# lucabaldesi/srsRAN

Measured on AMD Instinct MI355X. Metric: PDSCH decoded Mbps + code-blocks/sec, 20 MHz TM4 QAM256, 1/2/4/8 GPU, higher is better.
Workload: dtype fp32+int16; 1 GPU; srslte_ue_dl chain from time-domain I/Q: 2048 subframes/GPU/batch, 20 MHz (100 PRB), TM4 2x2 spatial multiplexing, 2 codewords QAM256 TBS 97896 (C=16, K=6144), MMSE+CSI, max 10 half-its with CRC early stop, 40 dB crossed 2x2 channel, every subframe distinct (GPU eNodeB generator, keyed by global subframe index); 3 PHY worker threads (own ue_dl / stream / softbuffers each) decode alternate batches,; subframes_per_gpu_batch=2048, code_blocks_per_gpu_batch=65536, workers_per_gpu=3, parallelism=dp1

## Files before the change

srsran_amd/csrc/tdec_kernels.hip:

```cpp
#include <hip/hip_runtime.h>

#include <atomic>
#include <stdint.h>
#include <stdlib.h>

#include "crc_device.h"
#include "tdec_internal.h"
#include "tdec_trellis.h"

namespace mi355 {

__device__ __forceinline__ uint32_t hi_lo(uint32_t a, uint32_t b) { return __builtin_amdgcn_alignbit(b, a, 16); }
__device__ __forceinline__ uint32_t from_prev(uint32_t v)
{
  return (uint32_t)__builtin_amdgcn_update_dpp(0, (int)v, 0x111, 0xf, 0xf, true);
}
__device__ __forceinline__ uint32_t from_next(uint32_t v)
{
  return (uint32_t)__builtin_amdgcn_update_dpp(0, (int)v, 0x101, 0xf, 0xf, true);
}

__device__ __forceinline__ void bm_set(uint32_t* bm, uint32_t m, bool v)
{
  __hip_atomic_fetch_or(&bm[m >> 5], (uint32_t)v << ((m & 31u) ^ 7u), __ATOMIC_RELAXED, __HIP_MEMORY_SCOPE_WORKGROUP);
}

template <int NL>
__device__ __forceinline__ void tdec_fused_check(const TdecWinArgs& a, int cb, int l, int K, const uint32_t* bm,
                                                 const uint32_t (*t4)[4][256])
{
  const DlschCheckArgs& c      = a.chk;
  const CbDesc&         d      = c.desc[cb];
  const uint32_t        nbytes = (uint32_t)K / 8, chunk = nbytes / NL;
  const int             pi     = d.C > 1 ? 1 : 0;
  const uint8_t*        bytes  = (const uint8_t*)bm;
  uint32_t              crc    = crc24_words(bytes + l * chunk, chunk, t4[pi]);
  crc = gf2_mulmod24(crc, c.scale[128 + 8 * pi + l], pi ? c.crc24b->poly : c.crc24a->poly);
#pragma unroll
  for (int o = NL / 2; o >= 1; o >>= 1) crc ^= (uint32_t)__shfl_xor((int)crc, o, 64);
  const bool ok  = crc == 0;
  const bool fin = ok || c.h + 1 == c.max_its;
  if (fin) {
    uint8_t*       dst  = c.data + d.data_off + (size_t)d.cb * d.rlen / 8;
    const uint32_t nb   = d.nb;
    const uint32_t head = min(nb, (4u - (uint32_t)((uintptr_t)dst & 3u)) & 3u);
    const uint32_t nw   = (nb - head) / 4, tail0 = head + 4 * nw;
    for (uint32_t i = l; i < head; i += NL) dst[i] = bytes[i];
    for (uint32_t i = tail0 + l; i < nb; i += NL) dst[i] = bytes[i];
    uint32_t* dw = (uint32_t*)(dst + head);
    const uint32_t sh = head;
    for (uint32_t w = l; w < nw; w += NL) {
      const uint32_t lo = bm[w + sh / 4], hi = bm[w + sh / 4 + 1];
      dw[w]             = sh ? __builtin_amdgcn_alignbyte(hi, lo, sh) : lo;
    }
    if (l == 0) {
      c.its[cb] = c.h + 1;
      if (ok) {
        c.done[cb]       = 1;
        c.sb_crc[d.slot] = 1;
      } else {
        c.done[cb] = 2;
      }
    }
  }
  const uint64_t un = __builtin_amdgcn_ballot_w64(l == 0 && !fin);
  if (un && (threadIdx.x & 63) == (uint32_t)__builtin_ctzll(un)) flag_set(c.next);
}


#define WG_AT(arr, j) (arr)[((size_t)grp * Lp + (j)) * 64 + q]

#define TDEC_BM_WORDS (8 * 193)
__shared__ uint32_t tdec_tx_lds[4][2][TDEC_SEG * 64];
__shared__ uint32_t tdec_ym_lds[4][8 * SB_ROWMASK_WORDS];
__shared__ uint32_t tdec_bm_lds[4 * TDEC_BM_WORDS];
__shared__ int16_t  tdec_stg_lds[4][TDEC_SEG * 128];
__shared__ uint32_t tdec_stg_row[4][TDEC_SEG];

#ifndef TDEC_WAVES_PER_EU
#define TDEC_WAVES_PER_EU 2
#endif
template <int NSB, int SEG, int MODE, int DIAG, bool FULL, int OUTK, bool GI = false, bool TX = false>
__device__ __forceinline__ void tdec_win_body(const TdecWinArgs& a, const int gl,
                                              const uint32_t (*crc_t4)[4][256] = nullptr)
{
  constexpr int NL = NSB / 2;
  constexpr int G  = 64 / NL;
  static_assert(!TX || (NSB == 16 && FULL && SEG == 8), "TX loads need 8-lane rows and whole 8-step segments");
  static_assert((DIAG >= 0 && DIAG <= 4) || DIAG == 20, "DIAG values the body knows");
  const int     grp = __builtin_amdgcn_readfirstlane(gl >> 6), q = gl & 63;
  const int     cbg = q / NL, l = q % NL;
  if constexpr (!TX) {
    if (grp * G + cbg >= a.ncb) return;
    if (a.done && a.done[grp * G + cbg]) return;
  }
  if (a.remaining && *a.remaining == 0) return;

  const int  L = a.L, Lp = a.Lp, nseg = a.nseg;
  constexpr bool CL     = DIAG == 20;
  constexpr bool dec2   = MODE == 2;
  constexpr bool has_ap = MODE == 1;

  const int       cb   = grp * G + cbg;
  const int       K    = L * NSB;
  const size_t    bidx = a.in_idx ? a.in_idx[cb] : (size_t)cb;
  const uint32_t* in32 = (const uint32_t*)(a.in + bidx * a.in_stride);
  const size_t    wg0  = (size_t)grp * Lp * 64 + q;
  const uint32_t* X    = dec2 ? a.E + wg0 : (GI ? a.gS + wg0 : in32 + l);
  const int       xs   = (dec2 || GI) ? 64 : NL;
  const uint32_t* Y    = GI ? a.gP + wg0 : in32 + (dec2 ? (K + 32) : (K + 32) / 2) + l;
  const int       ys   = GI ? 64 : NL;
  const uint32_t* AP   = a.A1 + wg0;
  uint32_t*       ck   = a.ckpt + (size_t)grp * nseg * 8 * 64 + q;

  const uint4*    txin  = nullptr;
  if constexpr (TX) {
    const int txc = grp * G + ((q >> 1) & 7);
    txin = (const uint4*)(a.in + (a.in_idx ? (size_t)a.in_idx[txc] : (size_t)txc) * a.in_stride) + (2 * (q >> 4) + (q & 1));
  }
  const int       txoX  = 0;
  const int       txoY  = (dec2 ? (L * NSB + 32) : (L * NSB + 32) / 2) / 4;
  uint32_t*       txb   = nullptr;
  if constexpr (TX) {
    txb = &tdec_tx_lds[threadIdx.x >> 6][0][0];
  }
  constexpr bool RMK = NSB == 16 && !GI;
  uint32_t*      ymask = nullptr;
  if constexpr (RMK) {
    ymask = tdec_ym_lds[threadIdx.x >> 6];
#pragma unroll
    for (int w = l; w < SB_ROWMASK_WORDS; w += NL) {
      uint32_t v = 0xffffffffu;
      if (a.rowmask) v = ((const uint32_t*)(a.in + bidx * a.in_stride + SB_ROWMASK))[(dec2 ? SB_ROWMASK_WORDS : 0) + w];
      ymask[cbg * SB_ROWMASK_WORDS + w] = v;
    }
    __builtin_amdgcn_fence(__ATOMIC_RELEASE, "wavefront");
    __builtin_amdgcn_wave_barrier();
    __builtin_amdgcn_fence(__ATOMIC_ACQUIRE, "wavefront");
  }
  auto yrow = [&](int c, int j) -> bool {
    if constexpr (RMK) {
      return (ymask[c * SB_ROWMASK_WORDS + (j >> 5)] >> (j & 31)) & 1u;
    } else {
      return true;
    }
  };
  auto tx_load = [&](int so, int j0, uint32_t* r, bool par = false) {
    const int    tc = (q >> 1) & 7, jr = j0 + (q >> 4);
    const uint4* p0 = txin + so + j0 * 2;
    const uint4* p1 = txin + so + (j0 + 4) * 2;
    if constexpr (RMK) {
      if (par) {
        p0 = yrow(tc, jr) ? p0 : a.zero16;
        p1 = yrow(tc, jr + 4) ? p1 : a.zero16;
      }
    }
    const uint4 v0 = *p0, v1 = *p1;
    if constexpr (dec2) {
      __builtin_memcpy(r, &v0, 16);
      __builtin_memcpy(r + 4, &v1, 16);
    } else {
      r[0] = v0.x; r[1] = v0.y; r[2] = v0.z; r[3] = v0.w;
      r[4] = v1.x; r[5] = v1.y; r[6] = v1.z; r[7] = v1.w;
    }
  };
  auto tx_unpack = [&](int b, const uint32_t* r, uint32_t* o) {
    uint32_t* w = txb + b * SEG * 64;
    if constexpr (dec2) {
      uint4 p0, p1;
      __builtin_memcpy(&p0, r, 16);
      __builtin_memcpy(&p1, r + 4, 16);
      ((uint4*)w)[q]      = p0;
      ((uint4*)w)[64 + q] = p1;
    } else {
      ((uint4*)w)[q]      = make_uint4(r[0], r[1], r[2], r[3]);
      ((uint4*)w)[64 + q] = make_uint4(r[4], r[5], r[6], r[7]);
    }
    __builtin_amdgcn_fence(__ATOMIC_RELEASE, "wavefront");
    __builtin_amdgcn_wave_barrier();
    __builtin_amdgcn_fence(__ATOMIC_ACQUIRE, "wavefront");
#pragma unroll
    for (int i = 0; i < SEG; i++) o[i] = w[64 * i + q];
  };

  v2s st[8], nw[8], aw[8];

  set_minf(aw);
#pragma unroll 1
  for (int b = 0; b < TDEC_WARMUP / 8; b++) {
    uint32_t xo[8], yo[8], ao[8] = {};
#pragma unroll
    for (int i = 0; i < 8; i++) {
      const int j = (L - TDEC_WARMUP) + 8 * b + i;
      xo[i]       = X[j * xs];
      yo[i]       = yrow(cbg, j) ? Y[j * ys] : 0u;
      if constexpr (has_ap) ao[i] = AP[j * 64];
    }
#pragma unroll
    for (int i = 0; i < 8; i++) {
      const int k = 8 * b + i;
      v2s       x = U(hi_lo(from_prev(xo[i]), xo[i]));
      if constexpr (has_ap) x = sadd(x, U(hi_lo(from_prev(ao[i]), ao[i])));
      if constexpr (CL) {
        aw[k & 7] = aw[k & 7] ^ x ^ U(yo[i]);
        continue;
      }
      v2s c0[8], c1[8];
      alpha_cands<true>(aw, x, U(hi_lo(from_prev(yo[i]), yo[i])), c0, c1);
#pragma unroll
      for (int s = 0; s < 8; s++) aw[s] = vmax(c0[s], c1[s]);
      if ((k & 1) == 0 && k != 0) normalize<true>(aw);
    }
  }

  if constexpr (DIAG != 2) {
  uint32_t cx[SEG], cy[SEG], ca[SEG] = {};
  auto     load = [&](int t, uint32_t* x, uint32_t* y, uint32_t* ap) {
    if constexpr (TX) {
      if constexpr (!dec2) tx_load(txoX, t * SEG, x);
      tx_load(txoY, t * SEG, y, true);
    }
#pragma unroll
    for (int i = 0; i < SEG; i++) {
      const int j = FULL ? t * SEG + i : min(t * SEG + i, L - 1);
      if constexpr (!TX || dec2) x[i] = X[j * xs];
      if constexpr (!TX) y[i] = yrow(cbg, j) ? Y[j * ys] : 0u;
      if constexpr (has_ap) ap[i] = AP[j * 64];
    }
  };
  uint32_t bx[SEG], by[SEG], ba[SEG] = {}, dx[SEG], dy[SEG], da[SEG] = {};
  load(nseg - 1, cx, cy, ca);
  load(max(nseg - 2, 0), bx, by, ba);
  set_minf(st);
#pragma unroll 1
  for (int b = TDEC_WARMUP / 8 - 1; b >= 0; b--) {
    uint32_t xo[8], yo[8], ao[8] = {};
#pragma unroll
    for (int i = 0; i < 8; i++) {
      const int j = 8 * b + i;
      xo[i]       = X[j * xs];
      yo[i]       = yrow(cbg, j) ? Y[j * ys] : 0u;
      if constexpr (has_ap) ao[i] = AP[j * 64];
    }
#pragma unroll
    for (int i = 7; i >= 0; i--) {
      const int k = 8 * b + i;
      v2s       x = U(hi_lo(xo[i], from_next(xo[i])));
      if constexpr (has_ap) x = sadd(x, U(hi_lo(ao[i], from_next(ao[i]))));
      if constexpr (CL) {
        st[k & 7] = st[k & 7] ^ x ^ U(yo[i]);
        continue;
      }
      beta_step<true>(st, x, U(hi_lo(yo[i], from_next(yo[i]))), nw);
#pragma unroll
      for (int s = 0; s < 8; s++) st[s] = nw[s];
      if ((k & 1) == 0 && k != 0) normalize<true>(st);
    }
  }
  if (l == NL - 1) {
    const int16_t* T = a.in + bidx * a.in_stride + 3 * (K + 32) + (dec2 ? 6 : 0);
    v2s            tr[8], tn[8];
    tr[0] = splat(0);
#pragma unroll
    for (int i = 1; i < 8; i++) tr[i] = splat(-TDEC_INF);
#pragma unroll
    for (int t = 2; t >= 0; t--) {
      beta_step<false>(tr, splat(T[2 * t]), splat(T[2 * t + 1]), tn);
#pragma unroll
      for (int i = 0; i < 8; i++) tr[i] = tn[i];
    }
#pragma unroll
    for (int i = 0; i < 8; i++) st[i] = (v2s){st[i].x, tr[i].y};
  }
#pragma unroll
  for (int s = 0; s < 8; s++) ck[((size_t)(nseg - 1) * 8 + s) * 64] = W(st[s]);

  {
    auto seg = [&](int t, bool pf, const uint32_t* rx, const uint32_t* ry, const uint32_t* sa, uint32_t* lx,
                   uint32_t* ly, uint32_t* la) {
      uint32_t sx[SEG], sy[SEG];
      __builtin_amdgcn_sched_barrier(0);
      if constexpr (TX) {
        if constexpr (!dec2) tx_unpack(0, rx, sx);
        tx_unpack(1, ry, sy);
      }
#pragma unroll
      for (int i = 0; i < SEG; i++) {
        if constexpr (!TX || dec2) sx[i] = rx[i];
        if constexpr (!TX) sy[i] = ry[i];
      }
      if (pf) load(max(t - 2, 0), lx, ly, la);
#pragma unroll
      for (int i = SEG - 1; i >= 0; i--) {
        const int k = t * SEG + i;
        if (FULL || k < L) {
          v2s x = U(sx[i]);
          if constexpr (has_ap) x = sadd(x, U(sa[i]));
          if constexpr (DIAG == 4) {
            st[0] = st[0] ^ x ^ U(sy[i]);
            continue;
          }
          if constexpr (CL) {
            st[i] = st[i] ^ x ^ U(sy[i]);
          } else {
            beta_step<true>(st, x, U(sy[i]), nw);
#pragma unroll
            for (int s = 0; s < 8; s++) st[s] = nw[s];
          }
          if (i == 0 && t > 0 && DIAG != 3) {
#pragma unroll
            for (int s = 0; s < 8; s++) ck[((size_t)(t - 1) * 8 + s) * 64] = W(st[s]);
          }
          if (!CL && (i & 1) == 0 && k != 0) normalize<true>(st);
        }
      }
    };
    int t = nseg - 1;
#pragma unroll 1
    for (; t >= 2; t -= 3) {
      seg(t, true, cx, cy, ca, dx, dy, da);
      seg(t - 1, true, bx, by, ba, cx, cy, ca);
      seg(t - 2, true, dx, dy, da, bx, by, ba);
    }
    if (t >= 0) seg(t, false, cx, cy, ca, dx, dy, da);
    if (t >= 1) seg(t - 1, false, bx, by, ba, cx, cy, ca);
  }
  }
  if constexpr (DIAG == 1 || DIAG == 3 || DIAG == 4) {
    if (st[0].x == 12345 && st[1].y == 777) a.D[q] = W(st[0]);
    return;
  }
#pragma unroll
  for (int s = 0; s < 8; s++) st[s] = aw[s];
  if (l == 0) {
    st[0].x = 0;
#pragma unroll
    for (int i = 1; i < 8; i++) st[i].x = -TDEC_INF;
  }

  int16_t*        E16  = (int16_t*)a.E + (size_t)grp * Lp * 128;
  int16_t*        A16  = (int16_t*)a.A1 + (size_t)grp * Lp * 128;
  int16_t*        D16  = (int16_t*)a.D + (size_t)grp * Lp * 128;
  const uint32_t* tab  = (dec2 ? a.dstA : a.dstE) + l;
  const int       lane0 = cbg * NL;
  constexpr bool  dec_o   = OUTK == 1 || OUTK == 3;
  constexpr bool  wr_bits = !dec2 && dec_o && FULL;
  constexpr bool  wr_bm   = dec_o && (dec2 || !FULL);
  constexpr bool  wr_d    = OUTK == 2;
  constexpr bool  wr_a1   = !(dec2 && OUTK == 3);
  constexpr bool  wr_e    = !(!dec2 && OUTK == 3);
  constexpr int BMW = NSB == 16 ? 193 : 25;
  uint32_t*     bm  = nullptr;
  if constexpr (dec2 || wr_bits || wr_bm) {
    static_assert(G * BMW <= TDEC_BM_WORDS, "decision bitmaps of a wave");
    bm = tdec_bm_lds + (threadIdx.x >> 6) * TDEC_BM_WORDS + cbg * BMW;
    if constexpr (wr_bm) {
      for (int w = l; w < K / 32; w += NL) bm[w] = 0;
      __builtin_amdgcn_fence(__ATOMIC_RELEASE, "wavefront");
      __builtin_amdgcn_wave_barrier();
    }
  }

  constexpr bool STG = FULL && !GI && (dec2 ? wr_a1 : wr_e);
  int16_t*       O16 = dec2 ? A16 : E16;
  int16_t*       stg = nullptr;
  uint32_t*      stg_row = nullptr;
  if constexpr (STG) {
    stg     = tdec_stg_lds[threadIdx.x >> 6];
    stg_row = tdec_stg_row[threadIdx.x >> 6];
  }
  auto put = [&](int i, uint32_t tb, v2s v) {
    if constexpr (STG) {
      stg[i * 128 + (tb & 127u) + 2 * lane0]         = v.x;
      stg[i * 128 + ((tb >> 16) & 127u) + 2 * lane0] = v.y;
      stg_row[i]                                     = (tb & 0xffffu) >> 7;
    } else {
      O16[(tb & 0xffffu) + lane0 * 2] = v.x;
      O16[(tb >> 16) + lane0 * 2]     = v.y;
    }
  };
  auto flush = [&]() {
    if constexpr (STG) {
      static_assert(SEG == 8 && NL % 4 == 0, "rows of 8 steps, whole 16-byte pieces per code block");
      constexpr int PPR = NL / 4;
      __builtin_amdgcn_fence(__ATOMIC_RELEASE, "wavefront");
      __builtin_amdgcn_wave_barrier();
      __builtin_amdgcn_fence(__ATOMIC_ACQUIRE, "wavefront");
#pragma unroll
      for (int k = 0; k < 2; k++) {
        const int      idx = k * NL + l, r = idx / PPR, pc = idx % PPR;
        const uint32_t jr  = stg_row[r];
        const uint4    v   = *(const uint4*)(stg + r * 128 + 2 * lane0 + pc * 8);
        *(uint4*)(O16 + (size_t)jr * 128 + 2 * lane0 + pc * 8) = v;
      }
      __builtin_amdgcn_fence(__ATOMIC_RELEASE, "wavefront");
      __builtin_amdgcn_wave_barrier();
    }
  };
  uint32_t cx[SEG], cy[SEG], ca[SEG] = {}, cd[SEG], cc[8];
  auto     load = [&](int t, uint32_t* x, uint32_t* y, uint32_t* ap, uint32_t* d, uint32_t* c) {
    if constexpr (TX) {
      if constexpr (!dec2) tx_load(txoX, t * SEG, x);
      tx_load(txoY, t * SEG, y, true);
    }
#pragma unroll
    for (int i = 0; i < SEG; i++) {
      const int j = FULL ? t * SEG + i : min(t * SEG + i, L - 1);
      if constexpr (!TX || dec2) x[i] = X[j * xs];
      if constexpr (!TX) y[i] = yrow(cbg, j) ? Y[j * ys] : 0u;
      if constexpr (has_ap) ap[i] = AP[j * 64];
      d[i] = tab[(size_t)j * NL];
    }
#pragma unroll
    for (int s = 0; s < 8; s++) c[s] = ck[((size_t)t * 8 + s) * 64];
  };
  load(0, cx, cy, ca, cd, cc);

  uint32_t nx[SEG], ny[SEG], na[SEG] = {}, nd[SEG], nc[8];
  auto fseg = [&](int t, const uint32_t* rx, const uint32_t* ry, const uint32_t* ca, const uint32_t* cd,
                  const uint32_t* cc, uint32_t* nx, uint32_t* ny, uint32_t* na, uint32_t* nd, uint32_t* nc) {
    uint32_t cx[SEG], cy[SEG];
    __builtin_amdgcn_sched_barrier(0);
    if constexpr (TX) {
      if constexpr (!dec2) tx_unpack(0, rx, cx);
      tx_unpack(1, ry, cy);
    }
#pragma unroll
    for (int i = 0; i < SEG; i++) {
      if constexpr (!TX || dec2) cx[i] = rx[i];
      if constexpr (!TX) cy[i] = ry[i];
    }
    const int s0 = t * SEG;
    const int e  = FULL ? s0 + SEG : ((s0 + SEG < L) ? s0 + SEG : L);
    uint32_t  bits = 0;
    load(min(t + 1, nseg - 1), nx, ny, na, nd, nc);

    v2s xin[SEG];
#pragma unroll
    for (int i = 0; i < SEG; i++) {
      if constexpr (has_ap) {
        xin[i] = sadd(U(cx[i]), U(ca[i]));
      } else {
        xin[i] = U(cx[i]);
      }
    }

    static_assert(SEG == 8, "the rebuild keeps the 8 rows of a segment in registers");
    v2s ck8[8];
#pragma unroll
    for (int s = 0; s < 8; s++) ck8[s] = U(cc[s]);
    if constexpr (CL) {
#pragma unroll
      for (int i = 0; i < SEG; i++) {
        const int j = s0 + i;
        if (FULL ? i < SEG : j < e) {
          const v2s      out = xin[i] ^ U(cy[i]) ^ ck8[i] ^ st[i];
          const uint32_t tb  = cd[i];
          if constexpr (!dec2) {
            if constexpr (wr_e) put(i, tb, out);
            bits |= ((uint32_t)(out.x > 0) << (15 - i)) | ((uint32_t)(out.y > 0) << (7 - i));
            if constexpr (wr_bm) {
              bm_set(bm, 2 * l * L + j, out.x > 0);
              bm_set(bm, (2 * l + 1) * L + j, out.y > 0);
            }
          } else {
            if constexpr (wr_a1) put(i, tb, out);
            if constexpr (wr_bm) {
              const uint32_t jd = (tb & 0xffffu) >> 7, wlo = tb & 15u, whi = (tb >> 16) & 15u;
              bm_set(bm, __umul24(wlo, (uint32_t)L) + jd, out.x > 0);
              bm_set(bm, __umul24(whi, (uint32_t)L) + jd, out.y > 0);
            }
          }
        }
      }
    } else {
      v2s        cur[8], R[8][8];
      const bool ck_norm = (e & 1) == 0 && e != L;
#pragma unroll
      for (int s = 0; s < 8; s++) cur[s] = ck8[s];
      if (ck_norm) normalize<true>(cur);
#pragma unroll
      for (int i = SEG; i >= 1; i--) {
        const int j = s0 + i;
        if (FULL ? i == SEG : j == e) {
#pragma unroll
          for (int s = 0; s < 8; s++) R[i - 1][s] = ck8[s];
        } else if (FULL ? i < SEG : j < e) {
          v2s row[8];
          beta_step<true>(cur, xin[i], U(cy[i]), row);
#pragma unroll
          for (int s = 0; s < 8; s++) cur[s] = row[s];
#pragma unroll
          for (int s = 0; s < 8; s++) R[i - 1][s] = row[s];
          if ((j & 1) == 0) normalize<true>(cur);
        }
      }
#pragma unroll
      for (int i = 0; i < SEG; i++) {
        const int j = s0 + i;
        if (FULL ? i < SEG : j < e) {
          v2s c0[8], c1[8];
          alpha_cands<true>(st, xin[i], U(cy[i]), c0, c1);
          v2s t0[8], t1[8];
#pragma unroll
          for (int s = 0; s < 8; s++) {
            t0[s] = sadd(R[i][s], c0[s]);
            t1[s] = sadd(R[i][s], c1[s]);
          }
          const v2s m0 = vmax(vmax(vmax(t0[0], t0[1]), vmax(t0[2], t0[3])), vmax(vmax(t0[4], t0[5]), vmax(t0[6], t0[7])));
          const v2s m1 = vmax(vmax(vmax(t1[0], t1[1]), vmax(t1[2], t1[3])), vmax(vmax(t1[4], t1[5]), vmax(t1[6], t1[7])));
          const v2s out = ssub(m1, m0);
#pragma unroll
          for (int s = 0; s < 8; s++) st[s] = vmax(c0[s], c1[s]);
          if ((i & 1) == 0 && j != 0) normalize<true>(st);

          const uint32_t tb  = cd[i];
          const uint32_t olo = (tb & 0xffffu) + lane0 * 2, ohi = (tb >> 16) + lane0 * 2;
          if constexpr (!dec2) {
            if constexpr (wr_e) put(i, tb, has_ap ? out - U(ca[i]) : out);
            if constexpr (wr_d) WG_AT(a.D, j) = W(out);
            bits |= ((uint32_t)(out.x > 0) << (15 - i)) | ((uint32_t)(out.y > 0) << (7 - i));
            if constexpr (wr_bm) {
              bm_set(bm, 2 * l * L + j, out.x > 0);
              bm_set(bm, (2 * l + 1) * L + j, out.y > 0);
            }
          } else {
            if constexpr (wr_a1) put(i, tb, out - xin[i]);
            if constexpr (wr_bm) {
              const uint32_t jd = (tb & 0xffffu) >> 7, wlo = tb & 15u, whi = (tb >> 16) & 15u;
              bm_set(bm, __umul24(wlo, (uint32_t)L) + jd, out.x > 0);
              bm_set(bm, __umul24(whi, (uint32_t)L) + jd, out.y > 0);
            }
            if constexpr (wr_d) {
              D16[olo] = out.x;
              D16[ohi] = out.y;
            }
          }
        }
      }
    }
    flush();
    if constexpr (wr_bits) {
      uint8_t* bb = (uint8_t*)bm + (size_t)(2 * l) * (L / 8) + t;
      bb[0]       = (uint8_t)(bits >> 8);
      bb[L / 8]   = (uint8_t)bits;
    }
  };
  __builtin_amdgcn_s_waitcnt(0x0f70);
#pragma unroll 1
  for (int t = 0; t < nseg; t += 2) {
    fseg(t, cx, cy, ca, cd, cc, nx, ny, na, nd, nc);
    if (t + 1 < nseg) fseg(t + 1, nx, ny, na, nd, nc, cx, cy, ca, cd, cc);
  }
  if constexpr (wr_bm || wr_bits) {
    __builtin_amdgcn_fence(__ATOMIC_RELEASE, "wavefront");
    __builtin_amdgcn_wave_barrier();
    __builtin_amdgcn_fence(__ATOMIC_ACQUIRE, "wavefront");
    if (crc_t4) {
      tdec_fused_check<NL>(a, cb, l, K, bm, crc_t4);
    } else {
      uint2* o = (uint2*)(a.dec + (size_t)cb * a.dec_stride);
      for (int w = l; w < K / 64; w += NL) o[w] = make_uint2(bm[2 * w], bm[2 * w + 1]);
    }
  }
}

template <int NSB, int SEG, int MODE, int DIAG = 0, bool FULL = false, int OUTK = 0, bool TX = false>
__global__ __launch_bounds__(256) __attribute__((amdgpu_waves_per_eu(TDEC_WAVES_PER_EU))) void tdec_win_halfit(TdecWinArgs a)
{
  const int gl = blockIdx.x * blockDim.x + threadIdx.x;
  const uint32_t (*t4)[4][256] = nullptr;
  if constexpr (OUTK == 1 || OUTK == 3) {
    __shared__ uint32_t crc_t4[2][4][256];
    if (a.chk_on) {
      if (a.remaining && *a.remaining == 0) return;
      const uint32_t ti = threadIdx.x;
      crc_t4[0][0][ti] = a.chk.crc24a->t[ti];
      crc_t4[1][0][ti] = a.chk.crc24b->t[ti];
      __syncthreads();
#pragma unroll
      for (int k = 1; k < 4; k++) {
        crc_t4[0][k][ti] = crc24_step_table(crc_t4[0][k - 1][ti], crc_t4[0][0]);
        crc_t4[1][k][ti] = crc24_step_table(crc_t4[1][k - 1][ti], crc_t4[1][0]);
        __syncthreads();
      }
      t4 = crc_t4;
    }
  }
  if constexpr (TX) {
    const int  cb  = (gl >> 6) * (128 / NSB) + (gl & 63) / (NSB / 2);
    const bool act = cb < a.ncb && !(a.done && a.done[cb]);
    if (__builtin_amdgcn_ballot_w64(act) == ~0ull) {
      tdec_win_body<NSB, SEG, MODE, DIAG, FULL, OUTK, false, true>(a, gl, t4);
      return;
    }
  }
  tdec_win_body<NSB, SEG, MODE, DIAG, FULL, OUTK>(a, gl, t4);
}


template <int NSB>
__global__ __launch_bounds__(256) void tdec_win_decide_rows(TdecDecideArgs a)
{
  constexpr int NL = NSB / 2;
  constexpr int G  = 64 / NL;
  const size_t  g  = (size_t)blockIdx.x * blockDim.x + threadIdx.x;
  const int     q  = (int)(g & 63);
  const size_t  r  = g >> 6;
  const int     nb = a.L / 8;
  const int     grp = (int)(r / nb), jb = (int)(r % nb);
  const int     cbg = q / NL, l = q % NL;
  const size_t  cb  = (size_t)grp * G + cbg;
  if (cb >= (size_t)a.ncb || (a.remaining && *a.remaining == 0) || (a.done && a.done[cb])) return;
  const uint32_t* D  = a.D + ((size_t)grp * a.Lp + 8 * jb) * 64 + q;
  uint32_t        lo = 0, hi = 0;
#pragma unroll
  for (int i = 0; i < 8; i++) {
    const v2s v = U(D[(size_t)i * 64]);
    lo |= (uint32_t)(v.x > 0) << (7 - i);
    hi |= (uint32_t)(v.y > 0) << (7 - i);
  }
  uint8_t* o = a.out + cb * a.out_stride;
  o[(2 * l) * nb + jb]     = (uint8_t)lo;
  o[(2 * l + 1) * nb + jb] = (uint8_t)hi;
}

template <int NSB>
__global__ __launch_bounds__(256) void tdec_win_decide(TdecDecideArgs a)
{
  constexpr int NL   = NSB / 2;
  constexpr int G    = 64 / NL;
  const size_t  g    = (size_t)blockIdx.x * blockDim.x + threadIdx.x;
  const int     K    = a.L * NSB;
  const int     nbyt = K / 8;
  const size_t  cb   = g / nbyt;
  if (cb >= (size_t)a.ncb || (a.remaining && *a.remaining == 0) || (a.done && a.done[cb])) return;
  const int      b   = (int)(g % nbyt);
  const int      grp = (int)(cb / G), cbg = (int)(cb % G);
  const int16_t* D16 = (const int16_t*)a.D + (size_t)grp * a.Lp * 128 + cbg * NL * 2;
  uint32_t       out = 0;
#pragma unroll
  for (int i = 0; i < 8; i++) {
    const int nat = 8 * b + i, w = nat / a.L, j = nat % a.L;
    out |= (uint32_t)(D16[(size_t)j * 128 + w] > 0) << (7 - i);
  }
  a.out[cb * a.out_stride + b] = (uint8_t)out;
}


static std::atomic<int> g_diag{-1};

static int diag_mode()
{
  int v = g_diag.load(std::memory_order_relaxed);
  if (v < 0) {
    const char* e = getenv("MI355_TDEC_DIAG");
    v             = e ? atoi(e) : 0;
    g_diag.store(v, std::memory_order_relaxed);
  }
  return v;
}

int tdec_set_diag(int mode)
{
  const int old = diag_mode();
  g_diag.store(mode < 0 ? 0 : mode, std::memory_order_relaxed);
  return old;
}

static size_t diag_lds()
{
  static const long m = getenv("MI355_TDEC_LDS") ? atol(getenv("MI355_TDEC_LDS")) : 0;
  return (size_t)m;
}

template <int NSB, int DIAG, bool FULL, int OUTK, bool TX = false>
static void launch_mode_t(int mode, int blocks, const TdecWinArgs& a, hipStream_t s)
{
  const size_t lds = diag_lds();
  if (mode == 0) {
    hipLaunchKernelGGL((tdec_win_halfit<NSB, TDEC_SEG, 0, DIAG, FULL, OUTK, TX>), dim3(blocks), dim3(256), lds, s, a);
  } else if (mode == 1) {
    hipLaunchKernelGGL((tdec_win_halfit<NSB, TDEC_SEG, 1, DIAG, FULL, OUTK, TX>), dim3(blocks), dim3(256), lds, s, a);
  } else {
    hipLaunchKernelGGL((tdec_win_halfit<NSB, TDEC_SEG, 2, DIAG, FULL, OUTK, TX>), dim3(blocks), dim3(256), lds, s, a);
  }
}

static bool tx_enabled()
{
  static const bool on = !getenv("MI355_TDEC_TX") || atoi(getenv("MI355_TDEC_TX")) != 0;
  return on;
}

template <int NSB, int DIAG, bool FULL, int OUTK>
static void launch_mode_o(int mode, int blocks, const TdecWinArgs& a, hipStream_t s)
{
  if constexpr (NSB == 16 && FULL && (DIAG == 0 || DIAG == 20)) {
    if (tx_enabled() && a.zero16 && (uintptr_t)a.in % 16 == 0 && (a.in_stride * sizeof(int16_t)) % 16 == 0 && (a.L * 16 + 32) % 16 == 0) {
      launch_mode_t<NSB, DIAG, FULL, OUTK, true>(mode, blocks, a, s);
      return;
    }
  }
  launch_mode_t<NSB, DIAG, FULL, OUTK>(mode, blocks, a, s);
}

template <int NSB, int DIAG, bool FULL = false>
static void launch_mode(int mode, int blocks, const TdecWinArgs& a, hipStream_t s)
{
  if constexpr (NSB == 16 && FULL && DIAG == 0) {
    if (a.dec && a.spec) {
      launch_mode_o<NSB, DIAG, FULL, 3>(mode, blocks, a, s);
      return;
    }
  }
  if (a.dec) {
    launch_mode_o<NSB, DIAG, FULL, 1>(mode, blocks, a, s);
  } else if (a.write_d) {
    launch_mode_o<NSB, DIAG, FULL, 2>(mode, blocks, a, s);
  } else {
    launch_mode_o<NSB, DIAG, FULL, 0>(mode, blocks, a, s);
  }
}

bool tdec_win_spec_ok(int nsb, int L) { return nsb == 16 && L % TDEC_SEG == 0 && diag_mode() == 0; }

hipError_t tdec_win_launch_halfit(int nsb, const TdecWinArgs& a, hipStream_t s)
{
  const int ngrp   = (a.ncb + (128 / nsb) - 1) / (128 / nsb);
  const int blocks = (ngrp * 64 + 255) / 256;
  const int mode   = (a.n & 1) ? 2 : (a.n > 0 ? 1 : 0);
  const int dm     = diag_mode();
  if (nsb == 16) {
    if (dm == 1) {
      launch_mode<16, 1>(mode, blocks, a, s);
    } else if (dm == 3) {
      launch_mode<16, 3>(mode, blocks, a, s);
    } else if (dm == 4) {
      launch_mode<16, 4>(mode, blocks, a, s);
    } else if (dm == 2) {
      launch_mode<16, 2>(mode, blocks, a, s);
    } else if (dm == 20 && a.L % TDEC_SEG == 0) {
      launch_mode<16, 20, true>(mode, blocks, a, s);
    } else if (a.L % TDEC_SEG == 0) {
      launch_mode<16, 0, true>(mode, blocks, a, s);
    } else {
      launch_mode<16, 0>(mode, blocks, a, s);
    }
  } else if (a.L % TDEC_SEG == 0) {
    launch_mode<8, 0, true>(mode, blocks, a, s);
  } else {
    launch_mode<8, 0>(mode, blocks, a, s);
  }
  return hipGetLastError();
}

hipError_t tdec_win_launch_decide(int nsb, const TdecDecideArgs& a, hipStream_t s)
{
  if (a.L % 8 == 0) {
    const int    G      = 128 / nsb;
    const size_t ngrp   = (a.ncb + G - 1) / G;
    const size_t total  = ngrp * (a.L / 8) * 64;
    const int    blocks = (int)((total + 255) / 256);
    if (nsb == 16) {
      hipLaunchKernelGGL(tdec_win_decide_rows<16>, dim3(blocks), dim3(256), 0, s, a);
    } else {
      hipLaunchKernelGGL(tdec_win_decide_rows<8>, dim3(blocks), dim3(256), 0, s, a);
    }
    return hipGetLastError();
  }
  const size_t total  = (size_t)a.ncb * (a.L * nsb / 8);
  const int    blocks = (int)((total + 255) / 256);
  if (nsb == 16) {
    hipLaunchKernelGGL(tdec_win_decide<16>, dim3(blocks), dim3(256), 0, s, a);
  } else {
    hipLaunchKernelGGL(tdec_win_decide<8>, dim3(blocks), dim3(256), 0, s, a);
  }
  return hipGetLastError();
}

}
```

Baseline: 129,000 Mbps.

## Interleave alpha and beta warmup with double-buffered prefetched loads

```diff
diff --git a/srsran_amd/csrc/tdec_kernels.hip b/srsran_amd/csrc/tdec_kernels.hip
--- a/srsran_amd/csrc/tdec_kernels.hip
+++ b/srsran_amd/csrc/tdec_kernels.hip
@@ -87,7 +87,7 @@
   constexpr int NL = NSB / 2;
   constexpr int G  = 64 / NL;
   static_assert(!TX || (NSB == 16 && FULL && SEG == 8), "TX loads need 8-lane rows and whole 8-step segments");
-  static_assert((DIAG >= 0 && DIAG <= 4) || DIAG == 20, "DIAG values the body knows");
+  static_assert((DIAG >= 0 && DIAG <= 6) || DIAG == 20, "DIAG values the body knows");
   const int     grp = __builtin_amdgcn_readfirstlane(gl >> 6), q = gl & 63;
   const int     cbg = q / NL, l = q % NL;
   if constexpr (!TX) {
@@ -185,95 +185,159 @@
 
   v2s st[8], nw[8], aw[8];
 
+  {
+  constexpr bool BWD = DIAG != 2;
+  auto load_at = [&](int j0, uint32_t* x, uint32_t* y, uint32_t* ap, bool UNC = false) {
+    if constexpr (TX) {
+      if constexpr (!dec2) tx_load(txoX, j0, x);
+      tx_load(txoY, j0, y, true);
+    }
+#pragma unroll
+    for (int i = 0; i < SEG; i++) {
+      const int j = FULL ? j0 + i : min(j0 + i, L - 1);
+      if constexpr (!TX || dec2) x[i] = X[j * xs];
+      if constexpr (!TX) {
+        if (UNC) {
+          const bool      has = yrow(cbg, j);
+          const uint32_t* py  = (!has && a.zero16) ? (const uint32_t*)a.zero16 : Y + j * ys;
+          const uint32_t  v   = *py;
+          y[i]                = has ? v : 0u;
+        } else {
+          y[i] = yrow(cbg, j) ? Y[j * ys] : 0u;
+        }
+      }
+      if constexpr (has_ap) ap[i] = AP[j * 64];
+    }
+  };
+  auto load = [&](int t, uint32_t* x, uint32_t* y, uint32_t* ap) { load_at(t * SEG, x, y, ap); };
+  auto take = [&](const uint32_t* rx, const uint32_t* ry, uint32_t* sx, uint32_t* sy) {
+    if constexpr (TX) {
+      if constexpr (!dec2) tx_unpack(0, rx, sx);
+      tx_unpack(1, ry, sy);
+      __builtin_amdgcn_fence(__ATOMIC_RELEASE, "wavefront");
+      __builtin_amdgcn_wave_barrier();
+    }
+#pragma unroll
+    for (int i = 0; i < SEG; i++) {
+      if constexpr (!TX || dec2) sx[i] = rx[i];
+      if constexpr (!TX) sy[i] = ry[i];
+    }
+  };
+  uint32_t cx[SEG], cy[SEG], ca[SEG] = {};
+  uint32_t bx[SEG], by[SEG], ba[SEG] = {}, dx[SEG], dy[SEG], da[SEG] = {};
+  auto     first_segments = [&]() {
+    if constexpr (BWD && DIAG != 5) {
+      load(nseg - 1, cx, cy, ca);
+      load(max(nseg - 2, 0), bx, by, ba);
+    }
+  };
+  int16_t tv[6] = {};
+  auto    tail_values = [&]() {
+    if constexpr (BWD) {
+      const int16_t* T = a.in + bidx * a.in_stride + 3 * (K + 32) + (dec2 ? 6 : 0);
+#pragma unroll
+      for (int i = 0; i < 6; i++) tv[i] = T[i];
+    }
+  };
   set_minf(aw);
-#pragma unroll 1
-  for (int b = 0; b < TDEC_WARMUP / 8; b++) {
-    uint32_t xo[8], yo[8], ao[8] = {};
-#pragma unroll
-    for (int i = 0; i < 8; i++) {
-      const int j = (L - TDEC_WARMUP) + 8 * b + i;
-      xo[i]       = X[j * xs];
-      yo[i]       = yrow(cbg, j) ? Y[j * ys] : 0u;
-      if constexpr (has_ap) ao[i] = AP[j * 64];
-    }
-#pragma unroll
-    for (int i = 0; i < 8; i++) {
-      const int k = 8 * b + i;
-      v2s       x = U(hi_lo(from_prev(xo[i]), xo[i]));
-      if constexpr (has_ap) x = sadd(x, U(hi_lo(from_prev(ao[i]), ao[i])));
-      if constexpr (CL) {
-        aw[k & 7] = aw[k & 7] ^ x ^ U(yo[i]);
-        continue;
-      }
-      v2s c0[8], c1[8];
-      alpha_cands<true>(aw, x, U(hi_lo(from_prev(yo[i]), yo[i])), c0, c1);
-#pragma unroll
-      for (int s = 0; s < 8; s++) aw[s] = vmax(c0[s], c1[s]);
-      if ((k & 1) == 0 && k != 0) normalize<true>(aw);
-    }
-  }
-
-  if constexpr (DIAG != 2) {
-  uint32_t cx[SEG], cy[SEG], ca[SEG] = {};
-  auto     load = [&](int t, uint32_t* x, uint32_t* y, uint32_t* ap) {
-    if constexpr (TX) {
-      if constexpr (!dec2) tx_load(txoX, t * SEG, x);
-      tx_load(txoY, t * SEG, y, true);
-    }
-#pragma unroll
-    for (int i = 0; i < SEG; i++) {
-      const int j = FULL ? t * SEG + i : min(t * SEG + i, L - 1);
-      if constexpr (!TX || dec2) x[i] = X[j * xs];
-      if constexpr (!TX) y[i] = yrow(cbg, j) ? Y[j * ys] : 0u;
-      if constexpr (has_ap) ap[i] = AP[j * 64];
-    }
-  };
-  uint32_t bx[SEG], by[SEG], ba[SEG] = {}, dx[SEG], dy[SEG], da[SEG] = {};
-  load(nseg - 1, cx, cy, ca);
-  load(max(nseg - 2, 0), bx, by, ba);
-  set_minf(st);
-#pragma unroll 1
-  for (int b = TDEC_WARMUP / 8 - 1; b >= 0; b--) {
-    uint32_t xo[8], yo[8], ao[8] = {};
-#pragma unroll
-    for (int i = 0; i < 8; i++) {
-      const int j = 8 * b + i;
-      xo[i]       = X[j * xs];
-      yo[i]       = yrow(cbg, j) ? Y[j * ys] : 0u;
-      if constexpr (has_ap) ao[i] = AP[j * 64];
-    }
-#pragma unroll
-    for (int i = 7; i >= 0; i--) {
-      const int k = 8 * b + i;
-      v2s       x = U(hi_lo(xo[i], from_next(xo[i])));
-      if constexpr (has_ap) x = sadd(x, U(hi_lo(ao[i], from_next(ao[i]))));
-      if constexpr (CL) {
-        st[k & 7] = st[k & 7] ^ x ^ U(yo[i]);
-        continue;
-      }
-      beta_step<true>(st, x, U(hi_lo(yo[i], from_next(yo[i]))), nw);
-#pragma unroll
-      for (int s = 0; s < 8; s++) st[s] = nw[s];
-      if ((k & 1) == 0 && k != 0) normalize<true>(st);
-    }
-  }
-  if (l == NL - 1) {
-    const int16_t* T = a.in + bidx * a.in_stride + 3 * (K + 32) + (dec2 ? 6 : 0);
-    v2s            tr[8], tn[8];
+  if constexpr (BWD) set_minf(st);
+  if constexpr (DIAG == 6) {
+    tail_values();
+    first_segments();
+  } else {
+    constexpr int NB = TDEC_WARMUP / 8;
+    uint32_t      wx[2][2][8], wy[2][2][8], wa[2][2][8] = {};
+    auto          wload = [&](int b, int s) {
+      load_at((L - TDEC_WARMUP) + 8 * b, wx[s][0], wy[s][0], wa[s][0], true);
+      if constexpr (BWD) load_at(8 * (NB - 1 - b), wx[s][1], wy[s][1], wa[s][1], true);
+    };
+    constexpr bool AHEAD = FULL || !has_ap;
+    if constexpr (AHEAD) wload(0, 0);
+    tail_values();
+#pragma unroll
+    for (int b = 0; b < NB; b++) {
+      const int rs = b & 1;
+      if constexpr (AHEAD) {
+        if (b + 1 < NB) wload(b + 1, rs ^ 1);
+      } else {
+        wload(b, rs);
+      }
+      if (b + 1 == NB) first_segments();
+      __builtin_amdgcn_sched_barrier(0);
+      uint32_t xo[8], yo[8];
+      take(wx[rs][0], wy[rs][0], xo, yo);
+      const uint32_t* ao = wa[rs][0];
+#pragma unroll
+      for (int i = 0; i < 8; i++) {
+        const int k = 8 * b + i;
+        v2s       x = U(hi_lo(from_prev(xo[i]), xo[i]));
+        if constexpr (has_ap) x = sadd(x, U(hi_lo(from_prev(ao[i]), ao[i])));
+        if constexpr (CL) {
+          aw[k & 7] = aw[k & 7] ^ x ^ U(yo[i]);
+          continue;
+        }
+        v2s c0[8], c1[8];
+        alpha_cands<true>(aw, x, U(hi_lo(from_prev(yo[i]), yo[i])), c0, c1);
+#pragma unroll
+        for (int s = 0; s < 8; s++) aw[s] = vmax(c0[s], c1[s]);
+        if ((k & 1) == 0 && k != 0) normalize<true>(aw);
+      }
+      if constexpr (BWD) {
+        uint32_t xb[8], yb[8];
+        take(wx[rs][1], wy[rs][1], xb, yb);
+        const uint32_t* ab = wa[rs][1];
+#pragma unroll
+        for (int i = 7; i >= 0; i--) {
+          const int k = 8 * (NB - 1 - b) + i;
+          v2s       x = U(hi_lo(xb[i], from_next(xb[i])));
+          if constexpr (has_ap) x = sadd(x, U(hi_lo(ab[i], from_next(ab[i]))));
+          if constexpr (CL) {
+            st[k & 7] = st[k & 7] ^ x ^ U(yb[i]);
+            continue;
+          }
+          beta_step<true>(st, x, U(hi_lo(yb[i], from_next(yb[i]))), nw);
+#pragma unroll
+          for (int s = 0; s < 8; s++) st[s] = nw[s];
+          if ((k & 1) == 0 && k != 0) normalize<true>(st);
+        }
+      }
+#pragma unroll
+      for (int s = 0; s < 8; s++) {
+        uint32_t w = W(aw[s]);
+        asm volatile("" : "+v"(w));
+        aw[s] = U(w);
+        if constexpr (BWD) {
+          uint32_t v = W(st[s]);
+          asm volatile("" : "+v"(v));
+          st[s] = U(v);
+        }
+      }
+      __builtin_amdgcn_sched_barrier(0);
+    }
+  }
+
+  if constexpr (BWD) {
+  {
+    v2s tr[8], tn[8];
     tr[0] = splat(0);
 #pragma unroll
     for (int i = 1; i < 8; i++) tr[i] = splat(-TDEC_INF);
 #pragma unroll
     for (int t = 2; t >= 0; t--) {
-      beta_step<false>(tr, splat(T[2 * t]), splat(T[2 * t + 1]), tn);
+      beta_step<false>(tr, splat(tv[2 * t]), splat(tv[2 * t + 1]), tn);
 #pragma unroll
       for (int i = 0; i < 8; i++) tr[i] = tn[i];
     }
-#pragma unroll
-    for (int i = 0; i < 8; i++) st[i] = (v2s){st[i].x, tr[i].y};
+    const bool last = l == NL - 1;
+#pragma unroll
+    for (int i = 0; i < 8; i++) st[i] = (v2s){st[i].x, last ? tr[i].y : st[i].y};
   }
 #pragma unroll
   for (int s = 0; s < 8; s++) ck[((size_t)(nseg - 1) * 8 + s) * 64] = W(st[s]);
+  if constexpr (DIAG == 5) {
+    if (st[0].x == 12345 && aw[1].y == 777) a.D[q] = W(st[0]) ^ W(aw[0]);
+    return;
+  }
 
   {
     auto seg = [&](int t, bool pf, const uint32_t* rx, const uint32_t* ry, const uint32_t* sa, uint32_t* lx,
@@ -324,6 +388,7 @@
     }
     if (t >= 0) seg(t, false, cx, cy, ca, dx, dy, da);
     if (t >= 1) seg(t - 1, false, bx, by, ba, cx, cy, ca);
+  }
   }
   }
   if constexpr (DIAG == 1 || DIAG == 3 || DIAG == 4) {
@@ -556,7 +621,9 @@
     __builtin_amdgcn_fence(__ATOMIC_RELEASE, "wavefront");
     __builtin_amdgcn_wave_barrier();
     __builtin_amdgcn_fence(__ATOMIC_ACQUIRE, "wavefront");
-    if (crc_t4) {
+    if constexpr (DIAG == 6) {
+      if (bm[l] == 0x12345677u && st[0].x == 12345) a.D[q] = W(st[0]);
+    } else if (crc_t4) {
       tdec_fused_check<NL>(a, cb, l, K, bm, crc_t4);
     } else {
       uint2* o = (uint2*)(a.dec + (size_t)cb * a.dec_stride);
@@ -696,7 +763,7 @@
 template <int NSB, int DIAG, bool FULL, int OUTK>
 static void launch_mode_o(int mode, int blocks, const TdecWinArgs& a, hipStream_t s)
 {
-  if constexpr (NSB == 16 && FULL && (DIAG == 0 || DIAG == 20)) {
+  if constexpr (NSB == 16 && FULL && (DIAG == 0 || DIAG == 5 || DIAG == 6 || DIAG == 20)) {
     if (tx_enabled() && a.zero16 && (uintptr_t)a.in % 16 == 0 && (a.in_stride * sizeof(int16_t)) % 16 == 0 && (a.L * 16 + 32) % 16 == 0) {
       launch_mode_t<NSB, DIAG, FULL, OUTK, true>(mode, blocks, a, s);
       return;
@@ -708,11 +775,19 @@
 template <int NSB, int DIAG, bool FULL = false>
 static void launch_mode(int mode, int blocks, const TdecWinArgs& a, hipStream_t s)
 {
-  if constexpr (NSB == 16 && FULL && DIAG == 0) {
+  if constexpr (NSB == 16 && FULL && (DIAG == 0 || DIAG == 5 || DIAG == 6)) {
     if (a.dec && a.spec) {
       launch_mode_o<NSB, DIAG, FULL, 3>(mode, blocks, a, s);
       return;
     }
+  }
+  if constexpr (DIAG == 5 || DIAG == 6) {
+    if (a.dec) {
+      launch_mode_o<NSB, DIAG, FULL, 1>(mode, blocks, a, s);
+    } else {
+      launch_mode<NSB, 0, FULL>(mode, blocks, a, s);
+    }
+    return;
   }
   if (a.dec) {
     launch_mode_o<NSB, DIAG, FULL, 1>(mode, blocks, a, s);
@@ -723,7 +798,11 @@
   }
 }
 
-bool tdec_win_spec_ok(int nsb, int L) { return nsb == 16 && L % TDEC_SEG == 0 && diag_mode() == 0; }
+bool tdec_win_spec_ok(int nsb, int L)
+{
+  const int dm = diag_mode();
+  return nsb == 16 && L % TDEC_SEG == 0 && (dm == 0 || dm == 5 || dm == 6);
+}
 
 hipError_t tdec_win_launch_halfit(int nsb, const TdecWinArgs& a, hipStream_t s)
 {
@@ -740,6 +819,10 @@
       launch_mode<16, 4>(mode, blocks, a, s);
     } else if (dm == 2) {
       launch_mode<16, 2>(mode, blocks, a, s);
+    } else if (dm == 5 && a.L % TDEC_SEG == 0) {
+      launch_mode<16, 5, true>(mode, blocks, a, s);
+    } else if (dm == 6 && a.L % TDEC_SEG == 0) {
+      launch_mode<16, 6, true>(mode, blocks, a, s);
     } else if (dm == 20 && a.L % TDEC_SEG == 0) {
       launch_mode<16, 20, true>(mode, blocks, a, s);
     } else if (a.L % TDEC_SEG == 0) {
```

Result: no change. 129,400 Mbps, median of 3 (+0.3%).
